# yukw777/EILEV

Hardware: AMD Instinct MI355X
Metric: clips/sec (8-frame, 16 in-context) encode+generate, eilev-blip2-opt-2.7b (higher is better)
Workload: dtype bf16

## Files before the change

### eilev_amd/csrc/common.h

```cpp
#pragma once
#include <hip/hip_runtime.h>
#include <stdint.h>

#include <type_traits>

#include "../../include/eilev.h"

typedef __bf16 bf16;
typedef __attribute__((ext_vector_type(8))) __bf16 bf16x8;
typedef __attribute__((ext_vector_type(4))) __bf16 bf16x4;
typedef __attribute__((ext_vector_type(2))) __bf16 bf16x2;
typedef __attribute__((ext_vector_type(4))) float f32x4;
typedef __attribute__((ext_vector_type(16))) float f32x16;

#define EILEV_HIP_CHECK(expr)                          \
    do {                                               \
        hipError_t _e = (expr);                        \
        if (_e != hipSuccess) return (int)_e;          \
    } while (0)

static inline int eilev_num_cu() {
    static int n = 0;
    if (!n) {
        int dev = 0, cu = 0;
// ... 192 lines not shown
    DBG_GEMM_FORCE_SHIFT = 4,
    DBG_GEMM_SKINNY_NO_PRELOAD = 1 << 7,
    DBG_GEMM_ROW_MAJOR_TILES = 1 << 8,
    DBG_GEMM_NO_EPILOGUE = 1 << 10,
    DBG_GEMM_NO_STORES = 1 << 11,
    DBG_GEMM_A_ROW0 = 1 << 12,
    DBG_GEMM_W_ROW0 = 1 << 13,
    DBG_GEMM_NO_WIDE = 1 << 14,
    DBG_GEMM_NO_STREAM_LAYOUT = 1 << 15,
    DBG_GEMM_C_ROW0 = 1 << 17,
    DBG_GEMM_NO_HALF_TILES = 1 << 19,
    DBG_GEMM_WIDE_TILED = 1 << 20,
    DBG_GEMM_NO_W6 = 1 << 21,
    DBG_GEMM_GROUP_SHIFT = 22,
    DBG_GEMM_PP4_NO_PRESTAGE = 1 << 24,
    DBG_GEMM_NB_SHIFT = 26,
    DBG_GEMM_ROWS32_FIRST_FIT = 1 << 27,
    DBG_GEMM_NO_ROWS32 = 1 << 28,
    DBG_GEMM_NO_REDUCE_LN = 1 << 29,
    DBG_GEMM_NB_BLOCKS_ONLY = 1 << 30,

    DBG_ATTN_NO_COMPUTE = 1 << 0,
    DBG_ATTN_NO_PREFETCH = 1 << 1,
    DBG_ATTN_NO_FRAME = 1 << 2,
    DBG_ATTN_FRAME3 = 1 << 4,
    DBG_ATTN_NO_FRAME3 = 1 << 5,
    DBG_ATTN_V2_4WAVES = 1 << 6,
    DBG_ATTN_FRAME_STAMPS = 1 << 8,
    DBG_ATTN_FRAME3_STAMPS = 1 << 9,
    DBG_ATTN_HEAD_MAJOR = 1 << 10,
    DBG_ATTN_FRAME3_NO_STORES = 1 << 11,
};
enum GemmForce : int { FORCE_NONE = 0, FORCE_PP4 = 9, FORCE_W6 = 12, FORCE_64x128 = 13, FORCE_128x128 = 14, FORCE_SPLIT_K = 15 };

struct GemmArgs {
    const bf16 *A;
    int64_t lda;
    const bf16 *W;
    int64_t ldw;
    const bf16 *Wp = nullptr;
    int a_frag = 0, c_frag = 0, ln_frag = 0;
    int hm_tok = 0, hm_heads = 0, hm_hd = 0;
    const bf16 *bias;
    const bf16 *resid;
    int64_t ldr;
    void *C;
    int64_t ldc;
// ... 19 lines not shown
    bf16 *ln_out = nullptr;
    float ln_eps = 0.0f;
    int k_slice = 0;
    unsigned long long *trace = nullptr;
    int trace_tiles = 0;
};

__host__ __device__ static inline int64_t frag32_index(int row, int col) { return (int64_t)(col >> 5) * 1024 + row * 32 + (col & 31); }

#ifdef EILEV_PROBES
extern int g_gemm_form;
#define GEMM_FORM(code) (g_gemm_form = (g_gemm_form & ~0xffff) | (code))
#define GEMM_FORM_BIT(bit) (g_gemm_form |= (bit))
extern int g_gemm_ks;
#define GEMM_FORM_KS(n) (g_gemm_ks = (n))
#else
#define GEMM_FORM(code) ((void)0)
#define GEMM_FORM_BIT(bit) ((void)0)
#define GEMM_FORM_KS(n) ((void)0)
#endif
enum : int { GEMM_FORM_ROW_CHUNKS = 1 << 16, GEMM_FORM_W8_EXPANDED = 1 << 17, GEMM_FORM_SPLIT_K = 1 << 18, GEMM_FORM_REDUCE_LN = 1 << 19,
             GEMM_FORM_STREAM_LAYOUT = 1 << 20 };

int launch_gemm(const GemmArgs &g, int prof_kind, hipStream_t s);
bool gemm_rows32_takes(const GemmArgs &g);
int launch_pp4_ext(const GemmArgs &g, int grid, hipStream_t s);
#ifdef EILEV_PROBES
#define EILEV_TRACE_M16 true
#else
#define EILEV_TRACE_M16 false
#endif
static inline bool pp4_all_lean(const GemmArgs &g) {
    const bool scale_ok = g.scale_cols == 0 || (g.scale_cols % 16 == 0 && g.epi == 0 && !g.resid && !g.ln_rows && !g.stat_out);
    return g.N % 128 == 0 && !g.out_f32 && g.patch_group == 0 && scale_ok && !g.wscale && !g.ascale && !g.dbg && (!g.trace || EILEV_TRACE_M16);
}
static inline bool hm_takes(const GemmArgs &g) {
    return g.hm_tok >= 128 && g.hm_heads > 0 && g.hm_hd > 64 && g.hm_hd % 8 == 0 && g.N == 3 * g.hm_heads * g.hm_hd && g.ln_rows && g.epi == 0 && !g.resid &&
           !g.stat_out && !g.scale_cols && pp4_all_lean(g) && g.N % 64 == 0 && g.M % g.hm_tok == 0 && (int64_t)g.M * g.N * 2 < 0xfffffff0ll;
}
bool gemv_rows_ok(int M, int N, int K);
int launch_gemv_rows(int pro, const bf16 *x, int64_t ldx, const bf16 *gamma, const bf16 *beta, float eps, const float *part, int heads, int hd,
                     int nsplit, const bf16 *W, const bf16 *bias, const bf16 *resid, int64_t ldr, void *out, int64_t ldo, int out_f32, int M, int N,
                     int K, int epi, float scale, int scale_cols, hipStream_t s);
bool gemv1_ok(int N, int K, int pro);
int launch_gemv1(int pro, const bf16 *x, const bf16 *gamma, const bf16 *beta, float eps, const bf16 *W, const bf16 *bias, const bf16 *resid, void *out,
                 int out_f32, int N, int K, int epi, float scale, int scale_cols, hipStream_t s, const float *part = nullptr, int heads = 0, int hd = 0,
                 int nsplit = 0);
bool gemvm_ok(int M, int N, int K, int pro);
int launch_gemvm(int pro, const bf16 *x, int64_t ldx, const bf16 *gamma, const bf16 *beta, float eps, const bf16 *W, const bf16 *bias, const bf16 *resid,
// ... 110 lines not shown
```

### eilev_amd/csrc/gemm.hip

```cpp
#include "gemm_common.h"
#include "gemm_tiled.h"
#include "gemm_pp4.h"
#include "gemm_w6.h"
#include "gemm_skinny.h"

int g_eilev_grid_cus = 0;
#ifdef EILEV_PROBES
int g_gemm_debug = 0;
extern "C" int eilev_debug_gemm_flags(int f) { g_gemm_debug = f; return 0; }
extern "C" int eilev_debug_grid_cus(int n) { g_eilev_grid_cus = n; return 0; }
int g_gemm_form = 0;
int g_gemm_ks = 0;
#endif
#ifdef EILEV_PROBES
unsigned long long *g_gemm_trace = nullptr;
int g_gemm_trace_tiles = 0;
extern "C" int eilev_debug_gemm_trace(void *buf, int tiles) { g_gemm_trace = (unsigned long long *)buf; g_gemm_trace_tiles = tiles; return 0; }
#endif

namespace {

#ifndef EILEV_A3_MIN_K
#define EILEV_A3_MIN_K 5120
#endif
bool a3_takes(const GemmArgs &g) { return g.epi == 0 && g.K >= EILEV_A3_MIN_K; }

int launch_pp4(const GemmArgs &g, hipStream_t s) {
    constexpr int smem = PP4_SMEM;
    const int tiles = ((g.M + 255) / 256) * ((g.N + 255) / 256);
    const int ncu = eilev_grid_cus();
    const int grid = tiles < ncu ? tiles : ncu / 8 * 8;
    if (g.A8 || g.ln_rows || g.stat_out) return launch_pp4_ext(g, grid, s);
    if (pp4_all_lean(g) && g.epi != 1) {
        if (a3_takes(g)) return GEMM_FORM(4030), eilev_launch<gemm_pp4_kernel<0, false, 0, 2, true>>(dim3(grid), dim3(512), smem, s, g);
        return eilev_with_epi<0, 2>(g.epi, [&](auto e) { return GEMM_FORM(4020 + decltype(e)::value), eilev_launch<gemm_pp4_kernel<decltype(e)::value, false, 0, 2>>(dim3(grid), dim3(512), smem, s, g); });
    }
    return eilev_with_epi<0, 1, 2>(g.epi, [&](auto e) { return GEMM_FORM(4000 + decltype(e)::value), eilev_launch<gemm_pp4_kernel<decltype(e)::value>>(dim3(grid), dim3(512), smem, s, g); });
}

constexpr int64_t kOffsetLimit = 0x7fff0000ll;
bool fits_offset(int64_t rows, int64_t ld) { return rows * ld * 2 < kOffsetLimit; }

GemmArgs with_probes(const GemmArgs &g_in) {
    GemmArgs g = g_in;
#ifdef EILEV_PROBES
    g.dbg = g_gemm_debug;
    g.trace = g_gemm_trace;
    g.trace_tiles = g_gemm_trace_tiles;
#else
// ... 132 lines not shown
    } else if (dma_ok) {
        GEMM_FORM(6100 + (m32 ? 20 : 10) + (pre ? 1 : 0));
        if (m32) rc = pre ? eilev_launch<gemm_skinny_dma_kernel<2, true>>(grid, dim3(256), 0, s, a) : eilev_launch<gemm_skinny_dma_kernel<2, false>>(grid, dim3(256), 0, s, a);
        else rc = pre ? eilev_launch<gemm_skinny_dma_kernel<1, true>>(grid, dim3(256), 0, s, a) : eilev_launch<gemm_skinny_dma_kernel<1, false>>(grid, dim3(256), 0, s, a);
    } else {
        GEMM_FORM(6000);
        rc = eilev_launch<gemm_skinny_kernel>(grid, dim3(256), 0, s, a);
    }
    if (rc != EILEV_OK || ks == 1) return rc;
    return skinny_reduce(g, a, s, ln_done);
}


bool pp4_takes(const GemmArgs &g) {
    return g.K % BK == 0 && g.patch_group == 0 && ceil_div64(g.M, 256) * ceil_div64(g.N, 256) >= 1024 &&
           (g.N >= 2048 || ceil_div64(g.M, 256) * ceil_div64(g.N, 128) >= 512) && fits_offset(g.N, g.ldw) && !g.dbg;
}

int64_t chunk_rows(const GemmArgs &g) {
    if (fits_offset(g.M, g.lda) || g.K % BK || g.patch_group || g.dbg || pp4_takes(g)) return 0;
    const int64_t rows = (kOffsetLimit / (g.lda * 2)) / 256 * 256;
    return rows >= 256 ? rows : 0;
}
int launch_row_chunks(const GemmArgs &g, int64_t rows_per, int prof_kind, hipStream_t s) {
    for (int64_t r0 = 0; r0 < g.M; r0 += rows_per) {
        GemmArgs c = g;
        c.M = (int)((g.M - r0) < rows_per ? (g.M - r0) : rows_per);
        c.A = g.A + r0 * g.lda;
        if (g.resid) c.resid = g.resid + r0 * g.ldr;
        if (g.stat_out) c.stat_out = g.stat_out + r0 * 2;
        if (g.ln_rows) c.ln_rows = g.ln_rows + r0 * 2;
        c.C = g.out_f32 ? (void *)(reinterpret_cast<float *>(g.C) + r0 * g.ldc) : (void *)(reinterpret_cast<bf16 *>(g.C) + r0 * g.ldc);
        c.ln_out = nullptr;
        const int rc = launch_gemm(c, prof_kind, s);
        if (rc != EILEV_OK) return rc;
// ... 156 lines not shown
    g.A = (const bf16 *)args->A; g.lda = args->lda; g.W = (const bf16 *)args->W; g.ldw = args->ldw;
    g.bias = (const bf16 *)args->bias; g.resid = (const bf16 *)args->resid; g.ldr = args->ldr; g.C = args->C; g.ldc = args->ldc;
    g.M = args->M; g.N = args->N; g.K = args->K; g.epi = args->epi; g.out_f32 = args->out_f32;
    g.scale = args->scale; g.scale_cols = args->scale_cols; g.patch_group = args->patch_group;
    g.hm_tok = args->hm_tok; g.hm_heads = args->hm_heads; g.hm_hd = args->hm_hd;
    g.wscale = args->wscale; g.W8 = (const uint8_t *)args->W8; g.w8_scratch = (bf16 *)args->w8_scratch;
    g.A8 = (const uint8_t *)args->A8; g.ascale = args->ascale; g.ln_rows = args->ln_rows; g.ln_csum = args->ln_csum;
    g.stat_out = args->stat_out; g.stat_ld = args->stat_ld;
    g.ln_gamma = (const bf16 *)args->ln_gamma; g.ln_beta = (const bf16 *)args->ln_beta; g.ln_out = (bf16 *)args->ln_out; g.ln_eps = args->ln_eps;
    return g;
}
extern "C" int eilev_debug_gemm(const EilevDebugGemmArgs *args, size_t struct_bytes, int *form, void *stream) {
    if (!args || struct_bytes != sizeof(EilevDebugGemmArgs)) return EILEV_E_BADARG;
    const GemmArgs g = debug_gemm_args(args);
    g_gemm_form = 0;
    const int rc = launch_gemm(g, -1, (hipStream_t)stream);
    if (form) *form = g_gemm_form;
    return rc;
}
struct EilevDebugSkinnyArgs {
    EilevDebugGemmArgs g;
    void *scratch; uint64_t scratch_bytes;
    const void *Wp;
    int32_t a_frag, c_frag, ln_frag, pad2;
};
extern "C" int eilev_debug_gemm_skinny(const EilevDebugSkinnyArgs *args, size_t struct_bytes, int *form, int *ks, void *stream) {
    if (!args || struct_bytes != sizeof(EilevDebugSkinnyArgs)) return EILEV_E_BADARG;
    GemmArgs g = debug_gemm_args(&args->g);
    g.scratch = (float *)args->scratch; g.scratch_bytes = (size_t)args->scratch_bytes; g.Wp = (const bf16 *)args->Wp;
    g.a_frag = args->a_frag; g.c_frag = args->c_frag; g.ln_frag = args->ln_frag;
// ... 9 lines not shown
```

### eilev_amd/csrc/gemm_pp4.h

```cpp
#pragma once
#include "gemm_common.h"

namespace {

#ifndef EILEV_PP4_DEEP
#define EILEV_PP4_DEEP 1
#endif
template <int EPI, bool F8 = false, int LN = 0, int M16K = 0, bool A3 = false>
__global__ __launch_bounds__(512, 2) void gemm_pp4_kernel(const GemmArgs g) {
    constexpr bool M16 = M16K != 0, HT16 = M16K == 2;
    constexpr bool TALL = HT16 && !A3;
    constexpr int TALL_BM = 384;
    constexpr int HT_WM = TALL ? TALL_BM / 4 : 64, HT_TM16 = HT_WM / 16;
    static_assert(!M16 || !F8, "16 x 16 form: bf16 instances");
    constexpr int BM = 256, BN = 256, NWM = 2, NWN = 4, NW = 8;
    constexpr int WM = BM / NWM, WN = BN / NWN, TM = WM / 32, TN = WN / 32;
    constexpr int STEP = (BM + BN) * 128;
    constexpr int PC = 8;
    static_assert(!A3 || M16, "A3: lean epilogues only");
    constexpr int STG0 = A3 ? 2 * BM * 128 : 2 * STEP;

    extern __shared__ __attribute__((aligned(16))) char smem[];
    auto a_slot = [&](int st) { return smem + (A3 ? (st % 3) * (BM * 128) : (st & 1) * STEP); };
    auto w_slot = [&](int st) { return smem + (A3 ? 3 * (BM * 128) + (st & 1) * (BN * 128) : (st & 1) * STEP + BM * 128); };
    const bool tall_n = TALL && (g.N & 255) == 128;
    const int tiles_m = (g.M + BM - 1) / BM, tiles_n = (g.N + BN - 1) / BN, ntiles = tall_n ? tall_ntiles(g.M, g.N) : tiles_m * tiles_n;
    const int tid = threadIdx.x, lane = tid & 63;
    const int wid = __builtin_amdgcn_readfirstlane(tid >> 6);
    const int wm = wid / NWN, wn = wid % NWN;
    const int l31 = lane & 31, hi = lane >> 5;
    const int l15 = lane & 15, g4 = lane >> 4;
    constexpr int TM16 = WM / 16, TN16 = WN / 16;
    const int ns = g.K / 64;
    const bool late = wid >= NW / 2;
    const int prow = lane >> 3, pslot = lane & 7;

    __amdgpu_buffer_rsrc_t ra = __builtin_amdgcn_make_buffer_rsrc((void *)g.A, 0, 0x7fffffff, 0x00020000);
    const __amdgpu_buffer_rsrc_t rw = __builtin_amdgcn_make_buffer_rsrc((void *)g.W, 0, 0x7fffffff, 0x00020000);
    unsigned po[PC];
    const int pw = late ? wid - NW / 2 : wid;
    bool src_a = !late;
    bool src_a_hi = !late;
    int d_lo = wid * (PC * 1024), d_hi = wid * (PC * 1024) + (PC / 2) * 1024;
    auto set_tile = [&](int t, int &m0, int &n0) {
        if (tall_n) {
            if constexpr (TALL) tile_coords_tall(g, m0, n0, t);
        } else {
            int tm_i, tn_i;
            tile_coords(g, tiles_m, tiles_n, tm_i, tn_i, t);
            m0 = tm_i * BM;
            n0 = tn_i * BN;
        }
        const bool tt = TALL && n0 + 128 >= g.N;
        src_a = !late || tt;
        src_a_hi = tt ? late : !late;
        if constexpr (TALL) {
            d_lo = tt ? (pw * HT_WM + (late ? 0 : 64)) * 128 : wid * (PC * 1024);
            d_hi = tt ? (late ? d_lo + (PC / 2) * 1024 : (TALL_BM + pw * 32) * 128) : d_lo + (PC / 2) * 1024;
        }
        {
#ifdef EILEV_PP4_PROBE_A0
            const uint64_t base = (uint64_t)(g.A);
#else
            const uint64_t base = (uint64_t)(g.A + (int64_t)m0 * g.lda);
#endif
            const uint64_t ub = ((uint64_t)(unsigned)__builtin_amdgcn_readfirstlane((int)(base >> 32)) << 32) |
                                (unsigned)__builtin_amdgcn_readfirstlane((int)(unsigned)base);
            ra = __builtin_amdgcn_make_buffer_rsrc((void *)ub, 0, 0x7fffffff, 0x00020000);
        }
#pragma unroll
        for (int i = 0; i < PC; ++i) {
            const int row = (!tt ? (pw * PC + i) * 8 : late ? pw * HT_WM + i * 8 : i < PC / 2 ? pw * HT_WM + 64 + i * 8 : pw * 32 + (i - PC / 2) * 8) + prow;
            const unsigned sw = (unsigned)((pslot ^ ((row >> 1) & 7)) << 4);
            if (i < PC / 2 ? src_a : src_a_hi) {
                int gr = m0 + row;
                gr = gr < g.M ? gr : g.M - 1;
                po[i] = (unsigned)(gr - m0) * (unsigned)(g.lda * 2) + sw;
            } else {
                int gr = n0 + row;
                gr = gr < g.N ? gr : g.N - 1;
                po[i] = (unsigned)gr * (unsigned)(g.ldw * 2) + sw;
            }
        }
    };
    auto stage_step = [&](int st, bool mine = true, int part = 0) {
        char *sd = (late ? w_slot(st) : a_slot(st)) + (pw * PC) * 1024;
        if (!mine) return;
#ifndef EILEV_PP4_PROBE_SKIP
#define EILEV_PP4_PROBE_SKIP 0
#endif
        constexpr int PCE = (EILEV_PP4_PROBE_SKIP & 4) ? 0 : (EILEV_PP4_PROBE_SKIP & 1) ? PC / 2 : PC;
        constexpr int PCL = (EILEV_PP4_PROBE_SKIP & 8) ? 0 : (EILEV_PP4_PROBE_SKIP & 2) ? PC / 2 : PC;
        if constexpr (TALL) {
            char *sb2 = smem + (st & 1) * STEP;
            auto issue4 = [&](int i0, bool from_a, char *dst) {
                if (from_a) {
#pragma unroll
                    for (int i = 0; i < PC / 2; ++i) __builtin_amdgcn_raw_ptr_buffer_load_lds(ra, (lds_void *)(dst + i * 1024), 16, po[i0 + i], st * 128, 0, 0);
                } else {
#pragma unroll
                    for (int i = 0; i < PC / 2; ++i) __builtin_amdgcn_raw_ptr_buffer_load_lds(rw, (lds_void *)(dst + i * 1024), 16, po[i0 + i], st * 128, 0, 0);
                }
            };
            if (part != 2) issue4(0, src_a, sb2 + d_lo);
            if (part != 1) issue4(PC / 2, src_a_hi, sb2 + d_hi);
        } else if (late) {
#pragma unroll
            for (int i = 0; i < PCL; ++i)
                if (part == 0 || (part == 1) == (i < PC / 2)) __builtin_amdgcn_raw_ptr_buffer_load_lds(rw, (lds_void *)(sd + i * 1024), 16, po[i], st * 128, 0, 0);
// ... 58 lines not shown
                for (int j = 0; j < TN16; ++j)
                    acc16[i][j] = __builtin_amdgcn_mfma_f32_16x16x32_bf16(bfr[j >> 1][j & 1], af[i >> 2][i & 3], acc16[i][j], 0, 0, 0);
        } else {
#pragma unroll
            for (int k2 = 0; k2 < 2; ++k2)
#pragma unroll
                for (int i = 0; i < TM; ++i)
#pragma unroll
                    for (int j = 0; j < TN; ++j)
                        acc[i][j] = __builtin_amdgcn_mfma_f32_32x32x16_bf16(bfr[k2][j], af[k2][i], acc[i][j], 0, 0, 0);
        }
        __builtin_amdgcn_s_setprio(0);
    };
    const int hm = TALL ? wid & 3 : wm * 2 + (wn >> 1), hn = TALL ? wid >> 2 : wn & 1;
    auto read_half_ht = [&](int st, int h) {
        const char *sa = a_slot(st) + (hm * HT_WM) * 128;
        const char *sb = (TALL ? a_slot(st) + TALL_BM * 128 : w_slot(st)) + (hn * 64) * 128;
        if constexpr (M16) {
            const int kc = h * 4 + g4;
#pragma unroll
            for (int j = 0; j < 4; ++j) {
                const int row = j * 16 + l15;
                bfr[j >> 1][j & 1] = *reinterpret_cast<const bf16x8 *>(sb + row * 128 + swz(row, kc));
            }
#pragma unroll
            for (int i = 0; i < HT_TM16; ++i) {
                const int row = i * 16 + l15;
                af[i >> 2][i & 3] = *reinterpret_cast<const bf16x8 *>(sa + row * 128 + swz(row, kc));
            }
            return;
        }
#pragma unroll
// ... 25 lines not shown
            for (int i = 0; i < HT_TM16; ++i)
#pragma unroll
                for (int j = 0; j < 4; ++j)
                    acc16[i][j] = __builtin_amdgcn_mfma_f32_16x16x32_bf16(bfr[j >> 1][j & 1], af[i >> 2][i & 3], acc16[i][j], 0, 0, 0);
        } else {
#pragma unroll
            for (int k2 = 0; k2 < 2; ++k2)
#pragma unroll
                for (int i = 0; i < 2; ++i)
#pragma unroll
                    for (int j = 0; j < 2; ++j)
                        acc[i][j] = __builtin_amdgcn_mfma_f32_32x32x16_bf16(bfr[k2][j], af[k2][i], acc[i][j], 0, 0, 0);
        }
        __builtin_amdgcn_s_setprio(0);
    };
    char *const stg = smem + STG0 + wid * 4096;
    const unsigned stg_sw = (unsigned)(STG0 + wid * 4096 + l31 * 128 + hi * 8) ^ (unsigned)((l31 & 7) << 4);
    const unsigned stg_sw16 = (unsigned)(STG0 + wid * 4096 + l15 * 128 + (g4 & 1) * 8) ^ (unsigned)((((g4 >> 1) ^ (l15 & 7)) << 4));
    const int srow = lane >> 3, schunk = lane & 7;
    auto is_lean = [&](int n0_) {
        return !(n0_ + 128 >= g.N && !(g.dbg & DBG_GEMM_NO_HALF_TILES)) && n0_ + BN <= g.N && !g.out_f32 && g.patch_group == 0 && g.scale_cols == 0 && !g.wscale && !g.ascale &&
               !(g.dbg & (DBG_GEMM_NO_EPILOGUE | DBG_GEMM_NO_STORES | DBG_GEMM_ROW0_STORES)) && !(g.dbg & DBG_GEMM_PP4_NO_PRESTAGE);
    };
    float ln_rs[LN == 1 ? (M16 ? TM16 : TM) : 1];
    auto lean_epilogue = [&](int cm0, int cn0, auto res_c, auto ht_c) {
        constexpr bool RES = decltype(res_c)::value;
        constexpr bool HTE = decltype(ht_c)::value;
        constexpr int NU = HTE ? HT_WM / 32 : TM;
        const int roff = HTE ? hm * HT_WM : wm * WM, coff = HTE ? hn * 64 : wn * WN;
        if constexpr (M16K == 1) {
            if (cn0 + coff >= g.N) return;
        }
        constexpr bool LNC = LN == 1 && !RES, LNP = LN == 2 && RES;
        typedef __attribute__((ext_vector_type(4))) unsigned u32x4_t;
        const int r0 = cm0 + roff;
        const int rows = g.M - r0 < 0 ? 0 : (g.M - r0 < NU * 32 ? g.M - r0 : NU * 32);
        auto uniform_rsrc = [&](const void *ptr, int bytes) {
            const uint64_t base = (uint64_t)ptr;
            const uint64_t ub = ((uint64_t)(unsigned)__builtin_amdgcn_readfirstlane((int)(base >> 32)) << 32) |
                                (unsigned)__builtin_amdgcn_readfirstlane((int)(unsigned)base);
            return __builtin_amdgcn_make_buffer_rsrc((void *)ub, 0, __builtin_amdgcn_readfirstlane(bytes), 0x00020000);
        };
        const __amdgpu_buffer_rsrc_t rc = uniform_rsrc(reinterpret_cast<bf16 *>(g.C) + (int64_t)r0 * g.ldc + cn0 + coff, rows * (int)(g.ldc * 2));
// ... 62 lines not shown
            float st1 = 0.0f, st2 = 0.0f;
            bf16x4 rcell[M16 ? 2 : TN][4];
            if constexpr (RES) {
#pragma unroll
                for (int it = 0; it < 4; ++it) {
                    const int row = it * 8 + srow;
                    *reinterpret_cast<u32x4_t *>(stg + row * 128 + ((schunk ^ (row & 7)) << 4)) = rv[it];
                }
                if constexpr (U + 1 < NU) res_load(U + 1);
                if constexpr (M16) {
#pragma unroll
                    for (int ib = 0; ib < 2; ++ib)
#pragma unroll
                        for (int j = 0; j < TN16; ++j) {
                            unsigned ca;
                            asm volatile("v_xor_b32 %0, %1, %2" : "=v"(ca) : "n"(((j * 2) << 4) | (ib << 11)), "v"(stg_sw16));
                            rcell[ib][j] = *reinterpret_cast<const bf16x4 *>(smem + ca);
                        }
                } else {
#pragma unroll
                for (int j = 0; j < TN; ++j)
#pragma unroll
                    for (int q = 0; q < 4; ++q) {
                        unsigned ca;
                        asm volatile("v_xor_b32 %0, %1, %2" : "=v"(ca) : "n"((j * 4 + q) << 4), "v"(stg_sw));
                        rcell[j][q] = *reinterpret_cast<const bf16x4 *>(smem + ca);
                    }
                }
            }
            float st16[2][2] = {{0.0f, 0.0f}, {0.0f, 0.0f}};
            if constexpr (M16) {
#pragma unroll
                for (int ib = 0; ib < 2; ++ib)
#pragma unroll
                    for (int j = 0; j < TN16; ++j) {
                        float v[4];
                        if constexpr (LNC) {
#pragma unroll
                            for (int e = 0; e < 4; ++e) v[e] = fmaf(acc16[2 * U + ib][j][e], ln_rs[2 * U + ib], (float)biasr16[j][e]);
                        } else {
// ... 11 lines not shown
                            for (int e = 0; e < 4; ++e) v[e] = fmaxf(v[e], 0.0f);
                        }
                        if constexpr (EPI == 1) gelu_erf_n<4>(v);
                        if constexpr (RES) {
#pragma unroll
                            for (int e = 0; e < 4; ++e) v[e] += (float)rcell[ib][j][e];
                        }
                        if constexpr (LNP) {
#pragma unroll
                            for (int e = 0; e < 4; ++e) {
                                st16[ib][0] += v[e];
                                st16[ib][1] = fmaf(v[e], v[e], st16[ib][1]);
                            }
                        }
                        unsigned ca;
                        asm volatile("v_xor_b32 %0, %1, %2" : "=v"(ca) : "n"(((j * 2) << 4) | (ib << 11)), "v"(stg_sw16));
                        *reinterpret_cast<bf16x4 *>(smem + ca) = (bf16x4){(bf16)v[0], (bf16)v[1], (bf16)v[2], (bf16)v[3]};
                    }
            } else {
#pragma unroll
            for (int j = 0; j < TN; ++j)
#pragma unroll
                for (int q = 0; q < 4; ++q) {
                    float v[4];
                    if constexpr (LNC) {
#pragma unroll
                        for (int e = 0; e < 4; ++e) v[e] = fmaf(acc[U][j][q * 4 + e], ln_rs[U], (float)biasr[j][q][e]);
                    } else {
#pragma unroll
                        for (int e = 0; e < 4; ++e) v[e] = acc[U][j][q * 4 + e] + (float)biasr[j][q][e];
                    }
// ... 2 lines not shown
                        for (int e = 0; e < 4; ++e) v[e] = fmaxf(v[e], 0.0f);
                    }
                    if constexpr (EPI == 1) gelu_erf_n<4>(v);
                    if constexpr (RES) {
#pragma unroll
                        for (int e = 0; e < 4; ++e) v[e] += (float)rcell[j][q][e];
                    }
                    if constexpr (LNP) {
#pragma unroll
                        for (int e = 0; e < 4; ++e) {
                            st1 += v[e];
                            st2 = fmaf(v[e], v[e], st2);
                        }
                    }
                    unsigned ca;
                    asm volatile("v_xor_b32 %0, %1, %2" : "=v"(ca) : "n"((j * 4 + q) << 4), "v"(stg_sw));
                    *reinterpret_cast<bf16x4 *>(smem + ca) = (bf16x4){(bf16)v[0], (bf16)v[1], (bf16)v[2], (bf16)v[3]};
                }
            }
            if constexpr (LNP && M16) {
                typedef __attribute__((ext_vector_type(2))) unsigned u32x2_t;
#pragma unroll
                for (int ib = 0; ib < 2; ++ib) {
                    float a1 = st16[ib][0], a2 = st16[ib][1];
                    a1 += __shfl_xor(a1, 16); a2 += __shfl_xor(a2, 16);
                    a1 += __shfl_xor(a1, 32); a2 += __shfl_xor(a2, 32);
                    const f32x2_t t = (f32x2_t){a1, a2};
                    if (g4 == 0) __builtin_amdgcn_raw_buffer_store_b64(__builtin_bit_cast(u32x2_t, t), rst, (U * 32 + ib * 16 + l15) * 8, 0, 0);
                }
            } else if constexpr (LNP) {
                typedef __attribute__((ext_vector_type(2))) unsigned u32x2_t;
// ... 33 lines not shown
#define PP_WAIT_VM0() __builtin_amdgcn_s_waitcnt(0x0F70)
#define PP_BARRIER()                       \
    do {                                   \
        __builtin_amdgcn_sched_barrier(0); \
        __builtin_amdgcn_s_barrier();      \
        __builtin_amdgcn_sched_barrier(0); \
    } while (0)

    int t = blockIdx.x, m0, n0;
    if (t >= ntiles) return;
    set_tile(t, m0, n0);
    auto w_piece_mine = [&](int n0_) { return TALL || !(n0_ + 128 >= g.N && !(g.dbg & DBG_GEMM_NO_HALF_TILES)) || wid < NW / 2 + 2; };
    stage_step(0, w_piece_mine(n0));
    bool pre1 = ns > 1 && (A3 || !(g.dbg & DBG_GEMM_PP4_NO_PRESTAGE));
    if (pre1) stage_step(1, w_piece_mine(n0));
    bool lean_cur = M16 || is_lean(n0);
    float ln_nm[LN == 1 ? (M16 ? TM16 : TM) : 1], ln_cl[LN == 1 ? (M16 ? TN16 : TN) : 1];
    auto ln_fetch = [&](int m0_, int n0_) {
        if constexpr (LN == 1 && M16) {
            const bool ht = HT16 && n0_ + 128 >= g.N;
            const int mb = m0_ + (ht ? hm * HT_WM : wm * WM) + l15, nb = n0_ + (ht ? hn * 64 : wn * WN) + l15;
            const __amdgpu_buffer_rsrc_t rl = __builtin_amdgcn_make_buffer_rsrc((void *)g.ln_rows, 0, g.M * 8, 0x00020000);
            const __amdgpu_buffer_rsrc_t rcs = __builtin_amdgcn_make_buffer_rsrc((void *)g.ln_csum, 0, g.N * 4, 0x00020000);
#pragma unroll
            for (int i = 0; i < TM16; ++i) ln_nm[i] = __builtin_bit_cast(float, __builtin_amdgcn_raw_buffer_load_b32(rl, (mb + i * 16) * 8 + 4, 0, 0));
#pragma unroll
            for (int j = 0; j < TN16; ++j) ln_cl[j] = __builtin_bit_cast(float, __builtin_amdgcn_raw_buffer_load_b32(rcs, (nb + j * 16) * 4, 0, 0));
        } else if constexpr (LN == 1) {
            const bool ht = n0_ + 128 >= g.N && !(g.dbg & DBG_GEMM_NO_HALF_TILES);
            const int mb = m0_ + (ht ? hm * 64 : wm * WM) + l31, nb = n0_ + (ht ? hn * 64 : wn * WN) + l31;
            const __amdgpu_buffer_rsrc_t rl = __builtin_amdgcn_make_buffer_rsrc((void *)g.ln_rows, 0, g.M * 8, 0x00020000);
            const __amdgpu_buffer_rsrc_t rcs = __builtin_amdgcn_make_buffer_rsrc((void *)g.ln_csum, 0, g.N * 4, 0x00020000);
#pragma unroll
            for (int i = 0; i < TM; ++i) ln_nm[i] = __builtin_bit_cast(float, __builtin_amdgcn_raw_buffer_load_b32(rl, (mb + i * 32) * 8 + 4, 0, 0));
#pragma unroll
            for (int j = 0; j < TN; ++j) ln_cl[j] = __builtin_bit_cast(float, __builtin_amdgcn_raw_buffer_load_b32(rcs, (nb + j * 32) * 4, 0, 0));
        }
    };
    ln_fetch(m0, n0);
    int trace_i = 0;
    const bool tracer = g.trace != nullptr && (wid == 0 || wid == NW / 2) && lane == 0;
#ifdef EILEV_PP4_ITRACE
#define ITR(k)                                                                                                              \
    do {                                                                                                                    \
        if (st == EILEV_PP4_ITRACE && tracer) *reinterpret_cast<volatile unsigned long long *>(stg + (k) * 8) = __builtin_amdgcn_s_memtime(); \
    } while (0)
#else
#define ITR(k) do { } while (0)
#endif
    auto stamp = [&](int k, bool core = false) {
#ifdef EILEV_PP4_ITRACE
        return;
#endif
        if (tracer && trace_i < g.trace_tiles)
            g.trace[(((size_t)blockIdx.x * 2 + (late ? 1 : 0)) * g.trace_tiles + trace_i) * 8 + k] =
                core ? __builtin_amdgcn_s_memtime() : __builtin_amdgcn_s_memrealtime();
    };
    for (; t < ntiles; t += gridDim.x) {
        stamp(0);
        stamp(5, true);
// ... 46 lines not shown
                for (int r = 0; r < 16; ++r) zero[r] = 0.0f;
#pragma unroll
                for (int i = 0; i < TM; ++i)
#pragma unroll
                    for (int j = 0; j < TN; ++j) acc[i][j] = __builtin_amdgcn_mfma_f32_32x32x8bf16_1k(ln_w1[j], ln_a1[i], zero, 0, 0, 0);
            } else {
#pragma unroll
                for (int i = 0; i < TM; ++i)
#pragma unroll
                    for (int j = 0; j < TN; ++j)
#pragma unroll
                        for (int r = 0; r < 16; ++r) acc[i][j][r] = 0.0f;
            }
        };
        if constexpr (LN != 1) acc_init();
        asm volatile("s_waitcnt vmcnt(0)" ::: "memory");
        PP_BARRIER();
        if (late) PP_BARRIER();
        stamp(1);
        const int nsd = (g.dbg & DBG_GEMM_ONE_KSTEP) ? 1 : ns;
        const bool half_tile = n0 + 128 >= g.N && !(g.dbg & DBG_GEMM_NO_HALF_TILES);
        auto kstep = [&](int st, auto first_c, auto ht_c) {
            constexpr bool FIRST = decltype(first_c)::value;
            constexpr bool HT = decltype(ht_c)::value;
            const bool w_mine = !HT || TALL || wid < NW / 2 + 2;
            ITR(0);
            if constexpr (HT) read_half_ht(st, 0); else read_half(st, 0);
#if EILEV_PP4_DEEP
#ifndef EILEV_PP4_SPLIT
#define EILEV_PP4_SPLIT 3
#endif
#ifndef EILEV_PP4_SPLIT_QKV
#define EILEV_PP4_SPLIT_QKV 0
#endif
            constexpr bool SPLIT_OK = (!HT || TALL) && (EILEV_PP4_SPLIT_QKV || !(LN == 1 && EPI == 0));
            constexpr bool SPLIT_E = (EILEV_PP4_SPLIT & 1) && SPLIT_OK, SPLIT_L = (EILEV_PP4_SPLIT & 2) && SPLIT_OK;
            if (!late) {
                if constexpr (A3) {
                    if (st + 2 < ns) stage_step(st + 2, w_mine, SPLIT_E ? 1 : 0);
                } else if (st + 1 < ns && !(FIRST && pre1)) stage_step(st + 1, w_mine, SPLIT_E ? 1 : 0);
            } else if (FIRST && !pre1 && ns > 1) stage_step(1, w_mine);
            else if (SPLIT_L && !FIRST && st + 1 < ns) stage_step(st + 1, w_mine, 2);
#else
            if (st + 1 < ns && !(FIRST && pre1)) stage_step(st + 1, w_mine);
#endif
            if constexpr (FIRST && LN == 1) acc_prep();
            PP_WAIT_LGKM0();
            ITR(1);
            PP_BARRIER();
            ITR(2);
            if constexpr (FIRST && LN == 1) acc_init();
            if constexpr (HT) mma_half_ht(); else mma_half();
            ITR(3);
            PP_BARRIER();
            ITR(4);
            if constexpr (HT) read_half_ht(st, 1); else read_half(st, 1);
#if EILEV_PP4_DEEP
            PP_WAIT_LGKM0();
            if (late) {
                PP_WAIT_VM0();
                if constexpr (!HT || TALL) if (st + 2 < ns) stage_step(st + 2, w_mine, SPLIT_L ? 1 : 0);
            } else if (A3) {
                if (SPLIT_E && st + 2 < ns) stage_step(st + 2, w_mine, 2);
            } else if (SPLIT_E && st + 1 < ns && !(FIRST && pre1)) stage_step(st + 1, w_mine, 2);
            ITR(5);
            PP_BARRIER();
            ITR(6);
            if constexpr (HT) {
                if constexpr (!TALL) if (late && st + 2 < ns) stage_step(st + 2, w_mine);
                mma_half_ht();
            } else mma_half();
            __builtin_amdgcn_sched_barrier(0);
            if constexpr (A3) {
                if (!late) {
                    if (st + 2 < ns) asm volatile("s_waitcnt vmcnt(8)" ::: "memory");
                    else asm volatile("s_waitcnt vmcnt(0)" ::: "memory");
                }
            } else if (!late) asm volatile("s_waitcnt vmcnt(0)" ::: "memory");
            ITR(7);
            PP_BARRIER();
#else
            PP_WAIT_LGKM0_VM0();
            PP_BARRIER();
            if constexpr (HT) mma_half_ht(); else mma_half();
            PP_BARRIER();
#endif
        };
        if (half_tile && M16K != 1) {
            if constexpr (M16K != 1) {
                kstep(0, std::true_type{}, std::true_type{});
                for (int st = 1; st < nsd; ++st) kstep(st, std::false_type{}, std::true_type{});
            }
        } else {
            kstep(0, std::true_type{}, std::false_type{});
            for (int st = 1; st < nsd; ++st) kstep(st, std::false_type{}, std::false_type{});
        }
        stamp(2);
#ifdef EILEV_PP4_ITRACE
        if (tracer && trace_i < g.trace_tiles) {
#pragma unroll
            for (int k = 0; k < 8; ++k)
                g.trace[(((size_t)blockIdx.x * 2 + (late ? 1 : 0)) * g.trace_tiles + trace_i) * 8 + k] = *reinterpret_cast<volatile unsigned long long *>(stg + k * 8);
        }
#endif
        if (!late) PP_BARRIER();
        if constexpr (LN == 1) {
            const __amdgpu_buffer_rsrc_t rl = __builtin_amdgcn_make_buffer_rsrc((void *)g.ln_rows, 0, g.M * 8, 0x00020000);
            if constexpr (M16) {
#pragma unroll
                for (int i = 0; i < TM16; ++i) ln_rs[i] = __builtin_bit_cast(float, __builtin_amdgcn_raw_buffer_load_b32(rl, (m0 + ((HT16 && half_tile) ? hm * HT_WM : wm * WM) + i * 16 + l15) * 8, 0, 0));
            } else {
#pragma unroll
            for (int u = 0; u < TM; ++u) ln_rs[u] = __builtin_bit_cast(float, __builtin_amdgcn_raw_buffer_load_b32(rl, (m0 + wm * WM + u * 32 + l31) * 8, 0, 0));
            }
        }
        const int cm0 = m0, cn0 = n0, tn = t + gridDim.x;
        const bool lean = lean_cur;
        pre1 = false;
        lean_cur = false;
        if (tn < ntiles) {
            set_tile(tn, m0, n0);
            stage_step(0, w_piece_mine(n0));
            pre1 = lean && ns > 1;
            if (pre1) stage_step(1, w_piece_mine(n0));
            lean_cur = M16 || is_lean(n0);
            ln_fetch(m0, n0);
        }
        stamp(3);
        if (HT16 && half_tile) {
            if constexpr (HT16) {
                if constexpr (LN == 1) lean_epilogue(cm0, cn0, std::false_type{}, std::true_type{});
                else if constexpr (LN == 2) lean_epilogue(cm0, cn0, std::true_type{}, std::true_type{});
                else if (g.resid != nullptr) lean_epilogue(cm0, cn0, std::true_type{}, std::true_type{});
                else lean_epilogue(cm0, cn0, std::false_type{}, std::true_type{});
            }
        } else if (lean || M16) {
            if constexpr (LN == 1) lean_epilogue(cm0, cn0, std::false_type{}, std::false_type{});
            else if constexpr (LN == 2) lean_epilogue(cm0, cn0, std::true_type{}, std::false_type{});
            else if (g.resid != nullptr) lean_epilogue(cm0, cn0, std::true_type{}, std::false_type{});
// ... 1 lines not shown
        } else if constexpr (!M16) {
            if (half_tile) {
                gemm_epilogue<64, 64, EPI, 0, 2, LN, true>(g, reinterpret_cast<f32x16(&)[2][2]>(acc), smem + STEP, cm0, cn0, hm, hn, wid, lane);
            } else {
                gemm_epilogue<WM, WN, EPI, 0, TM / 2, LN, true>(g, acc, smem + STEP, cm0, cn0, wm, wn, wid, lane);
                gemm_epilogue<WM, WN, EPI, TM / 2, TM, LN, true>(g, acc, smem + STEP, cm0, cn0, wm, wn, wid, lane);
            }
        }
        stamp(4);
        stamp(6, true);
        ++trace_i;
    }
#undef PP_BARRIER
}

constexpr int PP4_SMEM = 2 * 65536 + 8 * 4096;

}
```

### eilev_amd/csrc/gemm_pp4_ext.hip

```cpp
#include "gemm_pp4.h"

int launch_pp4_ext(const GemmArgs &g, int grid, hipStream_t s) {
    constexpr int smem = PP4_SMEM;
    if (g.A8 && g.hm_tok) return EILEV_E_UNSUPPORTED;
    if (g.A8) {
        if (g.epi == 1) return EILEV_E_UNSUPPORTED;
        GemmArgs h = g;
        h.A = reinterpret_cast<const bf16 *>(g.A8);
        h.W = reinterpret_cast<const bf16 *>(g.W8);
        h.K = g.K / 2; h.lda = g.lda / 2; h.ldw = g.ldw / 2;
        return eilev_with_epi<0, 2>(g.epi, [&](auto e) { return GEMM_FORM(4040 + decltype(e)::value), eilev_launch<gemm_pp4_kernel<decltype(e)::value, true>>(dim3(grid), dim3(512), smem, s, h); });
    }
    if (g.hm_tok && !hm_takes(g)) return EILEV_E_UNSUPPORTED;
    if (g.epi == 2 || g.out_f32 || (g.ln_rows && (g.resid || g.stat_out || !g.ln_csum || ((uintptr_t)g.ln_csum & 15) || ((uintptr_t)g.ln_rows & 7))) ||
        (g.stat_out && (!g.resid || g.epi != 0 || g.stat_ld < g.M || ((uintptr_t)g.stat_out & 7))))
        return EILEV_E_UNSUPPORTED;
    const bool lean = pp4_all_lean(g);
    if (g.stat_out)
        return GEMM_FORM(lean ? 4220 : 4200), lean ? eilev_launch<gemm_pp4_kernel<0, false, 2, 2>>(dim3(grid), dim3(512), smem, s, g)
                    : eilev_launch<gemm_pp4_kernel<0, false, 2>>(dim3(grid), dim3(512), smem, s, g);
    return eilev_with_epi<0, 1>(g.epi, [&](auto e) {
        constexpr int EPI = decltype(e)::value;
        return GEMM_FORM((lean ? 4110 : 4100) + EPI), lean ? eilev_launch<gemm_pp4_kernel<EPI, false, 1, 1>>(dim3(grid), dim3(512), smem, s, g)
                    : eilev_launch<gemm_pp4_kernel<EPI, false, 1>>(dim3(grid), dim3(512), smem, s, g);
    });
}
```

Baseline: 218.4.

## Extend three-deep A-operand ring staging to tall tiles and stats-epilogue GEMMs

Allows the A3 (three-slot A ring buffer) pipeline in the pp4 GEMM kernel to coexist with the tall 384-row tile form. Ring staging is used for regular tiles and double-buffered staging for tall/half tiles, with a re-stage step when the next tile's form differs. It also routes large-M, large-K residual+row-stats GEMMs to the A3 variant, and adds a debug bit that forces the route without disabling lean paths. The aim is deeper prefetch to hide global-load latency on long-K GEMMs. The cost is extra shared-memory slot bookkeeping, a staging barrier at form switches, and more template instances.

```diff
diff --git a/eilev_amd/csrc/common.h b/eilev_amd/csrc/common.h
--- a/eilev_amd/csrc/common.h
+++ b/eilev_amd/csrc/common.h
@@ -230,6 +230,7 @@
     DBG_GEMM_NO_W6 = 1 << 21,
     DBG_GEMM_GROUP_SHIFT = 22,
     DBG_GEMM_PP4_NO_PRESTAGE = 1 << 24,
+    DBG_GEMM_A3_RING = 1 << 25,
     DBG_GEMM_NB_SHIFT = 26,
     DBG_GEMM_ROWS32_FIRST_FIT = 1 << 27,
     DBG_GEMM_NO_ROWS32 = 1 << 28,
@@ -247,6 +248,7 @@
     DBG_ATTN_HEAD_MAJOR = 1 << 10,
     DBG_ATTN_FRAME3_NO_STORES = 1 << 11,
 };
+enum : int { DBG_GEMM_ROUTE_BITS = ~DBG_GEMM_A3_RING };
 enum GemmForce : int { FORCE_NONE = 0, FORCE_PP4 = 9, FORCE_W6 = 12, FORCE_64x128 = 13, FORCE_128x128 = 14, FORCE_SPLIT_K = 15 };
 
 struct GemmArgs {
@@ -296,10 +298,13 @@
 #define GEMM_FORM_BIT(bit) (g_gemm_form |= (bit))
 extern int g_gemm_ks;
 #define GEMM_FORM_KS(n) (g_gemm_ks = (n))
+extern int g_gemm_a_depth;
+#define GEMM_FORM_A_DEPTH(n) (g_gemm_a_depth = (n))
 #else
 #define GEMM_FORM(code) ((void)0)
 #define GEMM_FORM_BIT(bit) ((void)0)
 #define GEMM_FORM_KS(n) ((void)0)
+#define GEMM_FORM_A_DEPTH(n) ((void)0)
 #endif
 enum : int { GEMM_FORM_ROW_CHUNKS = 1 << 16, GEMM_FORM_W8_EXPANDED = 1 << 17, GEMM_FORM_SPLIT_K = 1 << 18, GEMM_FORM_REDUCE_LN = 1 << 19,
              GEMM_FORM_STREAM_LAYOUT = 1 << 20 };
@@ -314,7 +319,7 @@
 #endif
 static inline bool pp4_all_lean(const GemmArgs &g) {
     const bool scale_ok = g.scale_cols == 0 || (g.scale_cols % 16 == 0 && g.epi == 0 && !g.resid && !g.ln_rows && !g.stat_out);
-    return g.N % 128 == 0 && !g.out_f32 && g.patch_group == 0 && scale_ok && !g.wscale && !g.ascale && !g.dbg && (!g.trace || EILEV_TRACE_M16);
+    return g.N % 128 == 0 && !g.out_f32 && g.patch_group == 0 && scale_ok && !g.wscale && !g.ascale && !(g.dbg & DBG_GEMM_ROUTE_BITS) && (!g.trace || EILEV_TRACE_M16);
 }
 static inline bool hm_takes(const GemmArgs &g) {
     return g.hm_tok >= 128 && g.hm_heads > 0 && g.hm_hd > 64 && g.hm_hd % 8 == 0 && g.N == 3 * g.hm_heads * g.hm_hd && g.ln_rows && g.epi == 0 && !g.resid &&
diff --git a/eilev_amd/csrc/gemm.hip b/eilev_amd/csrc/gemm.hip
--- a/eilev_amd/csrc/gemm.hip
+++ b/eilev_amd/csrc/gemm.hip
@@ -11,6 +11,8 @@
 extern "C" int eilev_debug_grid_cus(int n) { g_eilev_grid_cus = n; return 0; }
 int g_gemm_form = 0;
 int g_gemm_ks = 0;
+int g_gemm_a_depth = 0;
+extern "C" int eilev_debug_gemm_a_depth(void) { return g_gemm_a_depth; }
 #endif
 #ifdef EILEV_PROBES
 unsigned long long *g_gemm_trace = nullptr;
@@ -20,9 +22,6 @@
 
 namespace {
 
-#ifndef EILEV_A3_MIN_K
-#define EILEV_A3_MIN_K 5120
-#endif
 bool a3_takes(const GemmArgs &g) { return g.epi == 0 && g.K >= EILEV_A3_MIN_K; }
 
 int launch_pp4(const GemmArgs &g, hipStream_t s) {
@@ -30,9 +29,10 @@
     const int tiles = ((g.M + 255) / 256) * ((g.N + 255) / 256);
     const int ncu = eilev_grid_cus();
     const int grid = tiles < ncu ? tiles : ncu / 8 * 8;
+    GEMM_FORM_A_DEPTH(2);
     if (g.A8 || g.ln_rows || g.stat_out) return launch_pp4_ext(g, grid, s);
     if (pp4_all_lean(g) && g.epi != 1) {
-        if (a3_takes(g)) return GEMM_FORM(4030), eilev_launch<gemm_pp4_kernel<0, false, 0, 2, true>>(dim3(grid), dim3(512), smem, s, g);
+        if (a3_takes(g)) return GEMM_FORM(4030), GEMM_FORM_A_DEPTH(3), eilev_launch<gemm_pp4_kernel<0, false, 0, 2, true>>(dim3(grid), dim3(512), smem, s, g);
         return eilev_with_epi<0, 2>(g.epi, [&](auto e) { return GEMM_FORM(4020 + decltype(e)::value), eilev_launch<gemm_pp4_kernel<decltype(e)::value, false, 0, 2>>(dim3(grid), dim3(512), smem, s, g); });
     }
     return eilev_with_epi<0, 1, 2>(g.epi, [&](auto e) { return GEMM_FORM(4000 + decltype(e)::value), eilev_launch<gemm_pp4_kernel<decltype(e)::value>>(dim3(grid), dim3(512), smem, s, g); });
@@ -195,11 +195,11 @@
 
 bool pp4_takes(const GemmArgs &g) {
     return g.K % BK == 0 && g.patch_group == 0 && ceil_div64(g.M, 256) * ceil_div64(g.N, 256) >= 1024 &&
-           (g.N >= 2048 || ceil_div64(g.M, 256) * ceil_div64(g.N, 128) >= 512) && fits_offset(g.N, g.ldw) && !g.dbg;
+           (g.N >= 2048 || ceil_div64(g.M, 256) * ceil_div64(g.N, 128) >= 512) && fits_offset(g.N, g.ldw) && !(g.dbg & DBG_GEMM_ROUTE_BITS);
 }
 
 int64_t chunk_rows(const GemmArgs &g) {
-    if (fits_offset(g.M, g.lda) || g.K % BK || g.patch_group || g.dbg || pp4_takes(g)) return 0;
+    if (fits_offset(g.M, g.lda) || g.K % BK || g.patch_group || (g.dbg & DBG_GEMM_ROUTE_BITS) || pp4_takes(g)) return 0;
     const int64_t rows = (kOffsetLimit / (g.lda * 2)) / 256 * 256;
     return rows >= 256 ? rows : 0;
 }
@@ -386,6 +386,7 @@
     if (!args || struct_bytes != sizeof(EilevDebugGemmArgs)) return EILEV_E_BADARG;
     const GemmArgs g = debug_gemm_args(args);
     g_gemm_form = 0;
+    g_gemm_a_depth = 0;
     const int rc = launch_gemm(g, -1, (hipStream_t)stream);
     if (form) *form = g_gemm_form;
     return rc;
diff --git a/eilev_amd/csrc/gemm_pp4.h b/eilev_amd/csrc/gemm_pp4.h
--- a/eilev_amd/csrc/gemm_pp4.h
+++ b/eilev_amd/csrc/gemm_pp4.h
@@ -9,7 +9,7 @@
 template <int EPI, bool F8 = false, int LN = 0, int M16K = 0, bool A3 = false>
 __global__ __launch_bounds__(512, 2) void gemm_pp4_kernel(const GemmArgs g) {
     constexpr bool M16 = M16K != 0, HT16 = M16K == 2;
-    constexpr bool TALL = HT16 && !A3;
+    constexpr bool TALL = HT16;
     constexpr int TALL_BM = 384;
     constexpr int HT_WM = TALL ? TALL_BM / 4 : 64, HT_TM16 = HT_WM / 16;
     static_assert(!M16 || !F8, "16 x 16 form: bf16 instances");
@@ -18,11 +18,12 @@
     constexpr int STEP = (BM + BN) * 128;
     constexpr int PC = 8;
     static_assert(!A3 || M16, "A3: lean epilogues only");
-    constexpr int STG0 = A3 ? 2 * BM * 128 : 2 * STEP;
+    constexpr int STG_RING = 2 * BM * 128, STG_DEEP2 = 2 * STEP;
+    constexpr int STG0 = A3 ? STG_RING : STG_DEEP2;
 
     extern __shared__ __attribute__((aligned(16))) char smem[];
-    auto a_slot = [&](int st) { return smem + (A3 ? (st % 3) * (BM * 128) : (st & 1) * STEP); };
-    auto w_slot = [&](int st) { return smem + (A3 ? 3 * (BM * 128) + (st & 1) * (BN * 128) : (st & 1) * STEP + BM * 128); };
+    auto a_slot = [&](int st, bool ring = A3) { return smem + (ring ? (st % 3) * (BM * 128) : (st & 1) * STEP); };
+    auto w_slot = [&](int st, bool ring = A3) { return smem + (ring ? 3 * (BM * 128) + (st & 1) * (BN * 128) : (st & 1) * STEP + BM * 128); };
     const bool tall_n = TALL && (g.N & 255) == 128;
     const int tiles_m = (g.M + BM - 1) / BM, tiles_n = (g.N + BN - 1) / BN, ntiles = tall_n ? tall_ntiles(g.M, g.N) : tiles_m * tiles_n;
     const int tid = threadIdx.x, lane = tid & 63;
@@ -41,7 +42,8 @@
     const int pw = late ? wid - NW / 2 : wid;
     bool src_a = !late;
     bool src_a_hi = !late;
-    int d_lo = wid * (PC * 1024), d_hi = wid * (PC * 1024) + (PC / 2) * 1024;
+    int d_lo = (A3 ? pw : wid) * (PC * 1024), d_hi = d_lo + (PC / 2) * 1024;
+    bool set_tall = false;
     auto set_tile = [&](int t, int &m0, int &n0) {
         if (tall_n) {
             if constexpr (TALL) tile_coords_tall(g, m0, n0, t);
@@ -54,8 +56,9 @@
         const bool tt = TALL && n0 + 128 >= g.N;
         src_a = !late || tt;
         src_a_hi = tt ? late : !late;
+        set_tall = tt;
         if constexpr (TALL) {
-            d_lo = tt ? (pw * HT_WM + (late ? 0 : 64)) * 128 : wid * (PC * 1024);
+            d_lo = tt ? (pw * HT_WM + (late ? 0 : 64)) * 128 : (A3 ? pw : wid) * (PC * 1024);
             d_hi = tt ? (late ? d_lo + (PC / 2) * 1024 : (TALL_BM + pw * 32) * 128) : d_lo + (PC / 2) * 1024;
         }
         {
@@ -83,7 +86,7 @@
             }
         }
     };
-    auto stage_step = [&](int st, bool mine = true, int part = 0) {
+    auto stage_step = [&](int st, bool mine = true, int part = 0, int form = -1) {
         char *sd = (late ? w_slot(st) : a_slot(st)) + (pw * PC) * 1024;
         if (!mine) return;
 #ifndef EILEV_PP4_PROBE_SKIP
@@ -92,7 +95,8 @@
         constexpr int PCE = (EILEV_PP4_PROBE_SKIP & 4) ? 0 : (EILEV_PP4_PROBE_SKIP & 1) ? PC / 2 : PC;
         constexpr int PCL = (EILEV_PP4_PROBE_SKIP & 8) ? 0 : (EILEV_PP4_PROBE_SKIP & 2) ? PC / 2 : PC;
         if constexpr (TALL) {
-            char *sb2 = smem + (st & 1) * STEP;
+            const bool deep2 = !A3 || (form < 0 ? set_tall : form != 0);
+            char *sb2 = deep2 ? smem + (st & 1) * STEP : late ? w_slot(st) : a_slot(st);
             auto issue4 = [&](int i0, bool from_a, char *dst) {
                 if (from_a) {
 #pragma unroll
@@ -181,8 +185,8 @@
     };
     const int hm = TALL ? wid & 3 : wm * 2 + (wn >> 1), hn = TALL ? wid >> 2 : wn & 1;
     auto read_half_ht = [&](int st, int h) {
-        const char *sa = a_slot(st) + (hm * HT_WM) * 128;
-        const char *sb = (TALL ? a_slot(st) + TALL_BM * 128 : w_slot(st)) + (hn * 64) * 128;
+        const char *sa = a_slot(st, false) + (hm * HT_WM) * 128;
+        const char *sb = (TALL ? a_slot(st, false) + TALL_BM * 128 : w_slot(st, false)) + (hn * 64) * 128;
         if constexpr (M16) {
             const int kc = h * 4 + g4;
 #pragma unroll
@@ -238,7 +242,6 @@
         }
         __builtin_amdgcn_s_setprio(0);
     };
-    char *const stg = smem + STG0 + wid * 4096;
     const unsigned stg_sw = (unsigned)(STG0 + wid * 4096 + l31 * 128 + hi * 8) ^ (unsigned)((l31 & 7) << 4);
     const unsigned stg_sw16 = (unsigned)(STG0 + wid * 4096 + l15 * 128 + (g4 & 1) * 8) ^ (unsigned)((((g4 >> 1) ^ (l15 & 7)) << 4));
     const int srow = lane >> 3, schunk = lane & 7;
@@ -251,6 +254,9 @@
         constexpr bool RES = decltype(res_c)::value;
         constexpr bool HTE = decltype(ht_c)::value;
         constexpr int NU = HTE ? HT_WM / 32 : TM;
+        constexpr int STG_D = (A3 && HTE) ? STG_DEEP2 - STG0 : 0;
+        char *const stg = smem + STG0 + STG_D + wid * 4096;
+        const unsigned sw = stg_sw + STG_D, sw16 = stg_sw16 + STG_D;
         const int roff = HTE ? hm * HT_WM : wm * WM, coff = HTE ? hn * 64 : wn * WN;
         if constexpr (M16K == 1) {
             if (cn0 + coff >= g.N) return;
@@ -343,7 +349,7 @@
 #pragma unroll
                         for (int j = 0; j < TN16; ++j) {
                             unsigned ca;
-                            asm volatile("v_xor_b32 %0, %1, %2" : "=v"(ca) : "n"(((j * 2) << 4) | (ib << 11)), "v"(stg_sw16));
+                            asm volatile("v_xor_b32 %0, %1, %2" : "=v"(ca) : "n"(((j * 2) << 4) | (ib << 11)), "v"(sw16));
                             rcell[ib][j] = *reinterpret_cast<const bf16x4 *>(smem + ca);
                         }
                 } else {
@@ -352,7 +358,7 @@
 #pragma unroll
                     for (int q = 0; q < 4; ++q) {
                         unsigned ca;
-                        asm volatile("v_xor_b32 %0, %1, %2" : "=v"(ca) : "n"((j * 4 + q) << 4), "v"(stg_sw));
+                        asm volatile("v_xor_b32 %0, %1, %2" : "=v"(ca) : "n"((j * 4 + q) << 4), "v"(sw));
                         rcell[j][q] = *reinterpret_cast<const bf16x4 *>(smem + ca);
                     }
                 }
@@ -394,7 +400,7 @@
                             }
                         }
                         unsigned ca;
-                        asm volatile("v_xor_b32 %0, %1, %2" : "=v"(ca) : "n"(((j * 2) << 4) | (ib << 11)), "v"(stg_sw16));
+                        asm volatile("v_xor_b32 %0, %1, %2" : "=v"(ca) : "n"(((j * 2) << 4) | (ib << 11)), "v"(sw16));
                         *reinterpret_cast<bf16x4 *>(smem + ca) = (bf16x4){(bf16)v[0], (bf16)v[1], (bf16)v[2], (bf16)v[3]};
                     }
             } else {
@@ -427,7 +433,7 @@
                         }
                     }
                     unsigned ca;
-                    asm volatile("v_xor_b32 %0, %1, %2" : "=v"(ca) : "n"((j * 4 + q) << 4), "v"(stg_sw));
+                    asm volatile("v_xor_b32 %0, %1, %2" : "=v"(ca) : "n"((j * 4 + q) << 4), "v"(sw));
                     *reinterpret_cast<bf16x4 *>(smem + ca) = (bf16x4){(bf16)v[0], (bf16)v[1], (bf16)v[2], (bf16)v[3]};
                 }
             }
@@ -491,6 +497,7 @@
     stage_step(0, w_piece_mine(n0));
     bool pre1 = ns > 1 && (A3 || !(g.dbg & DBG_GEMM_PP4_NO_PRESTAGE));
     if (pre1) stage_step(1, w_piece_mine(n0));
+    bool staged = true;
     bool lean_cur = M16 || is_lean(n0);
     float ln_nm[LN == 1 ? (M16 ? TM16 : TM) : 1], ln_cl[LN == 1 ? (M16 ? TN16 : TN) : 1];
     auto ln_fetch = [&](int m0_, int n0_) {
@@ -520,7 +527,7 @@
 #ifdef EILEV_PP4_ITRACE
 #define ITR(k)                                                                                                              \
     do {                                                                                                                    \
-        if (st == EILEV_PP4_ITRACE && tracer) *reinterpret_cast<volatile unsigned long long *>(stg + (k) * 8) = __builtin_amdgcn_s_memtime(); \
+        if (st == EILEV_PP4_ITRACE && tracer) *reinterpret_cast<volatile unsigned long long *>(stg_tr + (k) * 8) = __builtin_amdgcn_s_memtime(); \
     } while (0)
 #else
 #define ITR(k) do { } while (0)
@@ -597,6 +604,16 @@
             }
         };
         if constexpr (LN != 1) acc_init();
+        if constexpr (A3 && TALL) {
+            if (!staged) {
+                PP_WAIT_LGKM0_VM0();
+                PP_BARRIER();
+                stage_step(0);
+                pre1 = ns > 1;
+                if (pre1) stage_step(1);
+                staged = true;
+            }
+        }
         asm volatile("s_waitcnt vmcnt(0)" ::: "memory");
         PP_BARRIER();
         if (late) PP_BARRIER();
@@ -607,6 +624,11 @@
             constexpr bool FIRST = decltype(first_c)::value;
             constexpr bool HT = decltype(ht_c)::value;
             const bool w_mine = !HT || TALL || wid < NW / 2 + 2;
+            constexpr bool RING = A3 && !HT;
+            constexpr int FORM = HT ? 1 : 0;
+#ifdef EILEV_PP4_ITRACE
+            char *const stg_tr = smem + ((A3 && HT) ? STG_DEEP2 : STG0) + wid * 4096;
+#endif
             ITR(0);
             if constexpr (HT) read_half_ht(st, 0); else read_half(st, 0);
 #if EILEV_PP4_DEEP
@@ -619,11 +641,11 @@
             constexpr bool SPLIT_OK = (!HT || TALL) && (EILEV_PP4_SPLIT_QKV || !(LN == 1 && EPI == 0));
             constexpr bool SPLIT_E = (EILEV_PP4_SPLIT & 1) && SPLIT_OK, SPLIT_L = (EILEV_PP4_SPLIT & 2) && SPLIT_OK;
             if (!late) {
-                if constexpr (A3) {
-                    if (st + 2 < ns) stage_step(st + 2, w_mine, SPLIT_E ? 1 : 0);
-                } else if (st + 1 < ns && !(FIRST && pre1)) stage_step(st + 1, w_mine, SPLIT_E ? 1 : 0);
-            } else if (FIRST && !pre1 && ns > 1) stage_step(1, w_mine);
-            else if (SPLIT_L && !FIRST && st + 1 < ns) stage_step(st + 1, w_mine, 2);
+                if constexpr (RING) {
+                    if (st + 2 < ns) stage_step(st + 2, w_mine, SPLIT_E ? 1 : 0, FORM);
+                } else if (st + 1 < ns && !(FIRST && pre1)) stage_step(st + 1, w_mine, SPLIT_E ? 1 : 0, FORM);
+            } else if (FIRST && !pre1 && ns > 1) stage_step(1, w_mine, 0, FORM);
+            else if (SPLIT_L && !FIRST && st + 1 < ns) stage_step(st + 1, w_mine, 2, FORM);
 #else
             if (st + 1 < ns && !(FIRST && pre1)) stage_step(st + 1, w_mine);
 #endif
@@ -642,19 +664,19 @@
             PP_WAIT_LGKM0();
             if (late) {
                 PP_WAIT_VM0();
-                if constexpr (!HT || TALL) if (st + 2 < ns) stage_step(st + 2, w_mine, SPLIT_L ? 1 : 0);
-            } else if (A3) {
-                if (SPLIT_E && st + 2 < ns) stage_step(st + 2, w_mine, 2);
-            } else if (SPLIT_E && st + 1 < ns && !(FIRST && pre1)) stage_step(st + 1, w_mine, 2);
+                if constexpr (!HT || TALL) if (st + 2 < ns) stage_step(st + 2, w_mine, SPLIT_L ? 1 : 0, FORM);
+            } else if (RING) {
+                if (SPLIT_E && st + 2 < ns) stage_step(st + 2, w_mine, 2, FORM);
+            } else if (SPLIT_E && st + 1 < ns && !(FIRST && pre1)) stage_step(st + 1, w_mine, 2, FORM);
             ITR(5);
             PP_BARRIER();
             ITR(6);
             if constexpr (HT) {
-                if constexpr (!TALL) if (late && st + 2 < ns) stage_step(st + 2, w_mine);
+                if constexpr (!TALL) if (late && st + 2 < ns) stage_step(st + 2, w_mine, 0, FORM);
                 mma_half_ht();
             } else mma_half();
             __builtin_amdgcn_sched_barrier(0);
-            if constexpr (A3) {
+            if constexpr (RING) {
                 if (!late) {
                     if (st + 2 < ns) asm volatile("s_waitcnt vmcnt(8)" ::: "memory");
                     else asm volatile("s_waitcnt vmcnt(0)" ::: "memory");
@@ -681,9 +703,10 @@
         stamp(2);
 #ifdef EILEV_PP4_ITRACE
         if (tracer && trace_i < g.trace_tiles) {
+            char *const stg_tr = smem + ((A3 && HT16 && half_tile) ? STG_DEEP2 : STG0) + wid * 4096;
 #pragma unroll
             for (int k = 0; k < 8; ++k)
-                g.trace[(((size_t)blockIdx.x * 2 + (late ? 1 : 0)) * g.trace_tiles + trace_i) * 8 + k] = *reinterpret_cast<volatile unsigned long long *>(stg + k * 8);
+                g.trace[(((size_t)blockIdx.x * 2 + (late ? 1 : 0)) * g.trace_tiles + trace_i) * 8 + k] = *reinterpret_cast<volatile unsigned long long *>(stg_tr + k * 8);
         }
 #endif
         if (!late) PP_BARRIER();
@@ -703,9 +726,12 @@
         lean_cur = false;
         if (tn < ntiles) {
             set_tile(tn, m0, n0);
-            stage_step(0, w_piece_mine(n0));
-            pre1 = lean && ns > 1;
-            if (pre1) stage_step(1, w_piece_mine(n0));
+            if constexpr (A3 && TALL) staged = set_tall == half_tile;
+            if (staged) {
+                stage_step(0, w_piece_mine(n0));
+                pre1 = lean && ns > 1;
+                if (pre1) stage_step(1, w_piece_mine(n0));
+            }
             lean_cur = M16 || is_lean(n0);
             ln_fetch(m0, n0);
         }
@@ -737,6 +763,10 @@
 #undef PP_BARRIER
 }
 
+#ifndef EILEV_A3_MIN_K
+#define EILEV_A3_MIN_K 5120
+#endif
+
 constexpr int PP4_SMEM = 2 * 65536 + 8 * 4096;
 
 }
diff --git a/eilev_amd/csrc/gemm_pp4_ext.hip b/eilev_amd/csrc/gemm_pp4_ext.hip
--- a/eilev_amd/csrc/gemm_pp4_ext.hip
+++ b/eilev_amd/csrc/gemm_pp4_ext.hip
@@ -1,4 +1,11 @@
 #include "gemm_pp4.h"
+
+#ifndef EILEV_A3_STATS_MIN_M
+#define EILEV_A3_STATS_MIN_M 43776
+#endif
+static bool a3_stats_takes(const GemmArgs &g) {
+    return g.K >= EILEV_A3_MIN_K && (g.N % 256 == 128 || g.N % 256 == 0) && (g.M >= EILEV_A3_STATS_MIN_M || (g.dbg & DBG_GEMM_A3_RING));
+}
 
 int launch_pp4_ext(const GemmArgs &g, int grid, hipStream_t s) {
     constexpr int smem = PP4_SMEM;
@@ -16,6 +23,8 @@
         (g.stat_out && (!g.resid || g.epi != 0 || g.stat_ld < g.M || ((uintptr_t)g.stat_out & 7))))
         return EILEV_E_UNSUPPORTED;
     const bool lean = pp4_all_lean(g);
+    if (g.stat_out && lean && a3_stats_takes(g))
+        return GEMM_FORM(4220), GEMM_FORM_A_DEPTH(3), eilev_launch<gemm_pp4_kernel<0, false, 2, 2, true>>(dim3(grid), dim3(512), smem, s, g);
     if (g.stat_out)
         return GEMM_FORM(lean ? 4220 : 4200), lean ? eilev_launch<gemm_pp4_kernel<0, false, 2, 2>>(dim3(grid), dim3(512), smem, s, g)
                     : eilev_launch<gemm_pp4_kernel<0, false, 2>>(dim3(grid), dim3(512), smem, s, g);
```

Result: no change. 218.9 (median of 6 runs) (+0.3%).
